# alexgittens/libskylark

Measured on AMD Instinct MI355X. Metric: sketch+apply GB/s and randSVD wall-clock on 1e6×1e3 dense, 1/2/4/8 MI355X, higher is better.
Workload: dtype bf16; 1 GPU; model=FJLT + randomized rank-20 SVD (q=2) of dense bf16 1000000x1000, global_batch=1000000, seq_len=1000

## Files before the change

### libskylark_amd/_native/src/rsvd_engine.cpp

```cpp
#include <hip/hip_runtime.h>

#include <cstdlib>
#include <cstring>
#include <new>

#include "sl_common.hpp"

SL_API int sl_rsvd_pass_grid(int64_t m);
SL_API int64_t sl_rsvd_pass_workspace(int64_t m, int64_t n, int k);
SL_API int sl_rsvd_pass(const void* A, int64_t m, int64_t n, int64_t lda, const void* Zt, int k, void* ws, float* Y,
                        int64_t ldy, int final_pass, int variant, void* stream);
SL_API int sl_rsvd_reduce_z(const void* ws, int64_t m, int64_t n, int k, void* Wout, int w_f64, int ldw,
                            double* Gout, int ldg, int* zero_word, void* stream);
SL_API int sl_rsvd_make_v(const double* W, int n, int k, int ldw, const double* N, int r, float* V, const double* s64,
                          float* s32, void* stream);
SL_API int sl_rsvd_make_v_ind(const double* W, int n, int k, int ldw, const double* N, int r, const double* s64,
                              float* const* optr, void* stream);
SL_API int sl_rsvd_set_ptrs(float** tab, float* a, float* b, float* c, void* stream);
SL_API int64_t sl_rsvd_bnd_workspace(int k);
SL_API int sl_rsvd_bnd_coresident(int n, int k, int* ok);
SL_API int sl_rsvd_bnd_set_fault(const void* bws, int missing, uint64_t bound_ticks);
SL_API int sl_rsvd_boundary(int final_, int n, int k, int r, double* WG, void* bws, int* status, int status_or,
                            double* Rinv, void* Zt, float* M, double* N, double* s64, int* mirror, float* V,
                            float* s32, float* const* optr, void* stream);
SL_API int sl_tsk_f32_xm_ind(const float* Y, int64_t m, int k, const float* M, int k2, float* const* optr,
                             void* stream);
SL_API int sl_rsvd_fjlt_zt_tab(uint64_t seed, uint64_t baseD, uint64_t baseS, double scale, int k, int n, void* Zt,
                               float** tab, float* a, float* b, float* c, void* stream);
SL_API int sl_rsvd_fjlt_zt(uint64_t seed, uint64_t baseD, uint64_t baseS, double scale, int k, int n, void* Zt,
                           void* stream);
SL_API int sl_tsk_f32_xm(const float* Y, int64_t m, int k, int64_t ldy, const float* M, int k2, float* out,
                         int64_t ldo, double* G, void* ws, void* stream);
SL_API int sl_rsvd_zt_from_f64(const double* src, int64_t count, void* Zt, void* stream);
SL_API int sl_fill_random(void* out, int dtype, int dist, uint64_t seed, uint64_t base, int64_t rows, int64_t cols,
                          int64_t sr, int64_t sc, int64_t r0, int64_t c0, int64_t ir, int64_t ic, double p0, double p1,
                          double scale, int precise, void* stream);
SL_API int sl_comm_all_reduce(void* comm, const void* send, void* recv, int64_t count, int dtype, int op,
                              void* stream);

namespace {

struct Plan {
  int64_t m = 0, n = 0, lda = 0;
  int k = 0, r = 0, q = 0;
  char* base = nullptr;
  void* pass_ws = nullptr;
  uint16_t* Zt = nullptr;
  double* WG = nullptr;
  float* Y = nullptr;
  void* bnd_ws = nullptr;
  float* last_ptrs[3] = {nullptr, nullptr, nullptr};
  hipStream_t last_ptrs_stream = nullptr;
  bool fjlt_pending = false;
  uint64_t fj_seed = 0, fj_baseD = 0, fj_baseS = 0;
  double fj_scale = 0.0;
  double* Rinv = nullptr;
  float* M = nullptr;
  double* N = nullptr;
  double* s64 = nullptr;
  float** optr = nullptr;
  int* status = nullptr;
  int* mirror_host = nullptr;
  int* mirror_dev = nullptr;
  hipGraph_t graph[2] = {nullptr, nullptr};
  hipGraphExec_t exec[2] = {nullptr, nullptr};
  const void* graph_A = nullptr;
  hipStream_t cap_stream = nullptr;
  hipEvent_t cap_ev = nullptr;
};

int64_t align256(int64_t b) { return (b + 255) & ~(int64_t)255; }

int pass_nt_code() {
  static int c = -1;
  if (c < 0) {
    const char* e = std::getenv("SL_PASS_NT");
    c = e ? (std::atoi(e) & 7) : 0;
  }
  return c;
}

int pass_nt_final_code() {
  static int c = -1;
  if (c < 0) {
    const char* e = std::getenv("SL_PASS_NT_FINAL");
    c = e ? (std::atoi(e) & 7) : -1;
    if (c < 0) c = 8;
  }
  return c == 8 ? pass_nt_code() : c;
}

int flush_fjlt(Plan* p, hipStream_t s, float** tab = nullptr, float* a = nullptr, float* b = nullptr,
               float* c = nullptr) {
  if (!p->fjlt_pending) return SL_OK;
  p->fjlt_pending = false;
  return sl_rsvd_fjlt_zt_tab(p->fj_seed, p->fj_baseD, p->fj_baseS, p->fj_scale, p->k, (int)p->n, p->Zt, tab, a, b,
                             c, s);
}

int seg(Plan* p, const void* A, int i, hipStream_t s, float* V = nullptr, float* s32 = nullptr,
        float* const* optr = nullptr) {
  const bool final_pass = i == p->q;
  if (i > p->q + 1 || i < 0) { sl_set_last_error("rsvd: segment out of range"); return SL_ERR_INVALID; }
  int rc = SL_OK;
  if (i > 0) {
    const int fin = i == p->q + 1 ? 1 : 0;
    rc = sl_rsvd_boundary(fin, (int)p->n, p->k, p->r, p->WG, p->bnd_ws, p->status, 1, p->Rinv, p->Zt, p->M, p->N,
                          p->s64, p->mirror_dev, V, s32, optr, s);
    if (rc != SL_OK || fin) return rc;
  }
  rc = sl_rsvd_pass(A, p->m, p->n, p->lda, p->Zt, p->k, p->pass_ws, final_pass ? p->Y : nullptr, p->k,
                    final_pass ? 1 : 0, ((i & 1) ? 256 : 0) | ((final_pass ? pass_nt_final_code() : pass_nt_code()) << 9),
                    s);
  if (rc != SL_OK) return rc;
  return sl_rsvd_reduce_z(p->pass_ws, p->m, p->n, p->k, p->WG, 1, p->k, final_pass ? p->WG + p->n * p->k : nullptr,
                          p->k, i == 0 ? p->status : nullptr, s);
}

void drop_graph(Plan* p) {
  for (int v = 0; v < 2; ++v) {
    if (p->exec[v]) (void)hipGraphExecDestroy(p->exec[v]);
    if (p->graph[v]) (void)hipGraphDestroy(p->graph[v]);
    p->exec[v] = nullptr;
    p->graph[v] = nullptr;
  }
  p->graph_A = nullptr;
}

int finish_ind(Plan* p, hipStream_t s) {
  return sl_tsk_f32_xm_ind(p->Y, p->m, p->k, p->M, p->r, p->optr, s);
}

int capture(Plan* p, const void* A, int with_finish, hipStream_t st) {
  if (!p->cap_stream) {
    SL_HIP_CHECK(hipStreamCreateWithFlags(&p->cap_stream, hipStreamNonBlocking));
    SL_HIP_CHECK(hipEventCreateWithFlags(&p->cap_ev, hipEventDisableTiming));
  }
  SL_HIP_CHECK(hipEventRecord(p->cap_ev, st));
  SL_HIP_CHECK(hipStreamWaitEvent(p->cap_stream, p->cap_ev, 0));
  SL_HIP_CHECK(hipStreamSynchronize(p->cap_stream));
  hipStream_t cst = p->cap_stream;
  SL_HIP_CHECK(hipStreamBeginCapture(cst, hipStreamCaptureModeThreadLocal));
  int rc = SL_OK;
  for (int i = 0; i <= p->q + 1 && rc == SL_OK; ++i)
    rc = seg(p, A, i, cst, nullptr, nullptr, with_finish ? p->optr : nullptr);
  if (rc == SL_OK && with_finish) rc = finish_ind(p, cst);
  hipGraph_t g = nullptr;
  const hipError_t e = hipStreamEndCapture(cst, &g);
  if (rc != SL_OK || e != hipSuccess) {
    if (g) (void)hipGraphDestroy(g);
    if (rc == SL_OK) { sl_set_last_error(hipGetErrorString(e)); rc = SL_ERR_HIP; }
    return rc;
  }
  hipGraphExec_t ex = nullptr;
  if (hipGraphInstantiate(&ex, g, nullptr, nullptr, 0) != hipSuccess) {
    (void)hipGraphDestroy(g);
    sl_set_last_error("rsvd_run: graph instantiate failed");
    return SL_ERR_HIP;
  }
  p->graph[with_finish] = g;
  p->exec[with_finish] = ex;
  p->graph_A = A;
  return SL_OK;
}

}

SL_API int sl_rsvd_plan_create(int64_t m, int64_t n, int64_t lda, int k, int r, int q, void** out) {
  *out = nullptr;
  if (m < 1 || n < 16 || n > 1024 || n % 8 || lda % 8 || k < 1 || k > 48 || r < 1 || r > k || q < 0) {
    sl_set_last_error("rsvd_plan: needs m >= 1, 16 <= n <= 1024, n % 8 == 0, lda % 8 == 0, 1 <= r <= k <= 48, q >= 0");
    return SL_ERR_UNSUPPORTED;
  }
  {
    int ok = 0;
    const int rc = sl_rsvd_bnd_coresident((int)n, k, &ok);
    if (rc != SL_OK) return rc;
    if (!ok) return SL_ERR_UNSUPPORTED;
  }
  Plan* p = new (std::nothrow) Plan();
  if (!p) return SL_ERR_GENERIC;
  p->m = m; p->n = n; p->lda = lda; p->k = k; p->r = r; p->q = q;
  int64_t off = 0;
  const int64_t o_pass = off; off = align256(off + sl_rsvd_pass_workspace(m, n, k));
  const int64_t o_zt = off;   off = align256(off + n * k * 2);
  const int64_t o_wg = off;   off = align256(off + (n + k) * k * 8);
  const int64_t o_y = off;    off = align256(off + m * k * 4);
  const int64_t o_bnd = off;  off = align256(off + sl_rsvd_bnd_workspace(k));
  const int64_t o_ri = off;   off = align256(off + (int64_t)k * k * 8);
  const int64_t o_m = off;    off = align256(off + (int64_t)k * r * 4);
  const int64_t o_n = off;    off = align256(off + (int64_t)k * r * 8);
  const int64_t o_s = off;    off = align256(off + (int64_t)r * 8);
  const int64_t o_st = off;   off = align256(off + 16);
  const int64_t o_op = off;   off = align256(off + 4 * (int64_t)sizeof(float*));
  if (hipMalloc((void**)&p->base, (size_t)off) != hipSuccess) {
    delete p;
    sl_set_last_error("rsvd_plan: device allocation failed");
    return SL_ERR_HIP;
  }
  p->pass_ws = p->base + o_pass;
  p->Zt = (uint16_t*)(p->base + o_zt);
  p->WG = (double*)(p->base + o_wg);
  p->Y = (float*)(p->base + o_y);
  p->bnd_ws = p->base + o_bnd;
  p->Rinv = (double*)(p->base + o_ri);
  p->M = (float*)(p->base + o_m);
  p->N = (double*)(p->base + o_n);
  p->s64 = (double*)(p->base + o_s);
  p->status = (int*)(p->base + o_st);
  p->optr = (float**)(p->base + o_op);
  if (hipMemset(p->bnd_ws, 0, (size_t)sl_rsvd_bnd_workspace(k)) != hipSuccess ||
      hipMemset(p->status, 0, 16) != hipSuccess) {
    (void)hipFree(p->base);
    delete p;
    sl_set_last_error("rsvd_plan: memset failed");
    return SL_ERR_HIP;
  }
  if (hipHostMalloc((void**)&p->mirror_host, 64, hipHostMallocMapped) == hipSuccess) {
    *p->mirror_host = 0;
    if (hipHostGetDevicePointer((void**)&p->mirror_dev, p->mirror_host, 0) != hipSuccess) {
      (void)hipHostFree(p->mirror_host);
      p->mirror_host = p->mirror_dev = nullptr;
    }
  }
  *out = p;
  return SL_OK;
}

SL_API int sl_rsvd_plan_destroy(void* plan) {
  Plan* p = (Plan*)plan;
  if (!p) return SL_OK;
  drop_graph(p);
  (void)sl_rsvd_bnd_set_fault(p->bnd_ws, 0, 0);
  if (p->cap_ev) (void)hipEventDestroy(p->cap_ev);
  if (p->cap_stream) (void)hipStreamDestroy(p->cap_stream);
  if (p->mirror_host) (void)hipHostFree(p->mirror_host);
  (void)hipFree(p->base);
  delete p;
  return SL_OK;
}

SL_API int sl_rsvd_plan_bind(void* plan, double* WG, int* status) {
  Plan* p = (Plan*)plan;
  drop_graph(p);
  if (WG) p->WG = WG;
  if (status) p->status = status;
  return SL_OK;
}

SL_API int sl_rsvd_plan_set_fault(void* plan, int missing, uint64_t bound_ticks) {
  Plan* p = (Plan*)plan;
  drop_graph(p);
  return sl_rsvd_bnd_set_fault(p->bnd_ws, missing, bound_ticks);
}

SL_API int sl_rsvd_set_fjlt(void* plan, uint64_t seed, uint64_t baseD, uint64_t baseS, double scale, void* stream) {
  (void)stream;
  Plan* p = (Plan*)plan;
  p->fjlt_pending = true;
  p->fj_seed = seed; p->fj_baseD = baseD; p->fj_baseS = baseS; p->fj_scale = scale;
  return SL_OK;
}

SL_API int sl_rsvd_set_dense(void* plan, int dist, uint64_t seed, uint64_t base, double p0, double p1, double scale,
                             void* stream) {
  Plan* p = (Plan*)plan;
// ... 107 lines not shown
```

### libskylark_amd/_native/src/rsvd_pass.hip

```cpp
#include <algorithm>

#include "sl_common.hpp"

namespace {

typedef __attribute__((ext_vector_type(8))) __bf16 bf16x8;
typedef __attribute__((ext_vector_type(4))) short s16x4;
typedef __attribute__((ext_vector_type(8))) short s16x8;
typedef __attribute__((ext_vector_type(4))) float f32x4;
typedef __attribute__((ext_vector_type(4))) double f64x4;
typedef __attribute__((address_space(3))) void lds_void;
typedef __attribute__((address_space(3))) s16x4 lds_s16x4;


__device__ __forceinline__ void glds16(const void* gsrc, unsigned lds_base) {
  unsigned keep;
  asm volatile(
      "s_mov_b32 %0, m0\n\t"
      "s_mov_b32 m0, %2\n\t"
      "s_nop 0\n\t"
      "global_load_lds_dwordx4 %1, off\n\t"
      "s_mov_b32 m0, %0"
      : "=&s"(keep)
      : "v"(gsrc), "s"(lds_base)
      : "memory");
}

template <bool NT = false>
__device__ __forceinline__ void glds16s(unsigned voff, const void* sbase, unsigned lds_base) {
  unsigned keep;
  if constexpr (NT)
    asm volatile(
        "s_mov_b32 %0, m0\n\t"
        "s_mov_b32 m0, %3\n\t"
        "s_nop 0\n\t"
        "global_load_lds_dwordx4 %1, %2 nt\n\t"
        "s_mov_b32 m0, %0"
        : "=&s"(keep)
        : "v"(voff), "s"(sbase), "s"(lds_base)
        : "memory");
  else
    asm volatile(
        "s_mov_b32 %0, m0\n\t"
        "s_mov_b32 m0, %3\n\t"
        "s_nop 0\n\t"
        "global_load_lds_dwordx4 %1, %2\n\t"
        "s_mov_b32 m0, %0"
        : "=&s"(keep)
        : "v"(voff), "s"(sbase), "s"(lds_base)
        : "memory");
}

__device__ __forceinline__ void wait_vm(int n) {
  switch (n) {
#define SLW(N) case N: asm volatile("s_waitcnt vmcnt(" #N ")" ::: "memory"); break;
    SLW(0) SLW(1) SLW(2) SLW(3) SLW(4) SLW(5) SLW(6) SLW(7) SLW(8) SLW(9) SLW(10) SLW(11) SLW(12) SLW(13)
    SLW(14) SLW(15) SLW(16) SLW(17) SLW(18) SLW(19) SLW(20) SLW(21) SLW(22) SLW(23) SLW(24) SLW(25)
    SLW(26) SLW(27) SLW(28) SLW(29) SLW(30) SLW(31)
#undef SLW
    default: asm volatile("s_waitcnt vmcnt(0)" ::: "memory"); break;
  }
}

__device__ __forceinline__ void lds_barrier() {
  asm volatile("s_waitcnt lgkmcnt(0)" ::: "memory");
  __builtin_amdgcn_s_barrier();
  asm volatile("" ::: "memory");
}

template <int NCH>
__device__ __forceinline__ int swz4(int row) {
  if constexpr (NCH == 16) return ((row << 1) & 15) ^ (((row >> 3) & 1) * 9);
  else return row & (NCH - 1);
}


template <typename IT, typename OT>
__device__ __forceinline__ void reduce_body(const IT* __restrict__ slab, int nslab, int64_t total, int cols,
                                            OT* __restrict__ out, int ldo, int blk, double (*part)[128]) {
  const int lane = threadIdx.x & 63, v = threadIdx.x >> 6;
  const int64_t e0 = (int64_t)blk * 128 + 2 * lane;
  double a0 = 0, a1 = 0, b0 = 0, b1 = 0;
  if (e0 + 1 < total) {
    int s = v;
    for (; s + 56 < nslab; s += 64) {
      IT x0[8], x1[8];
#pragma unroll
      for (int q = 0; q < 8; ++q) {
        const IT* p = slab + (int64_t)(s + 8 * q) * total + e0;
        x0[q] = p[0];
        x1[q] = p[1];
      }
#pragma unroll
      for (int q = 0; q < 8; q += 2) {
        a0 += (double)x0[q]; a1 += (double)x1[q];
        b0 += (double)x0[q + 1]; b1 += (double)x1[q + 1];
      }
    }
    for (; s + 8 < nslab; s += 16) {
      const IT* p = slab + (int64_t)s * total + e0;
      const IT* q = p + 8 * total;
      a0 += (double)p[0]; a1 += (double)p[1];
      b0 += (double)q[0]; b1 += (double)q[1];
    }
    for (; s < nslab; s += 8) {
      const IT* p = slab + (int64_t)s * total + e0;
      a0 += (double)p[0]; a1 += (double)p[1];
    }
  } else if (e0 < total) {
    for (int s = v; s < nslab; s += 8) a0 += (double)slab[(int64_t)s * total + e0];
  }
  part[v][2 * lane] = a0 + b0;
  part[v][2 * lane + 1] = a1 + b1;
  __syncthreads();
  if (threadIdx.x < 128) {
    const int64_t e = (int64_t)blk * 128 + threadIdx.x;
    if (e < total) {
      double sum = 0;
#pragma unroll
      for (int u = 0; u < 8; ++u) sum += part[u][threadIdx.x];
      const int64_t i = e / cols, j = e - i * cols;
      out[i * ldo + j] = (OT)sum;
    }
  }
}

template <typename IT, typename OT>
__global__ void __launch_bounds__(512)
k_rsvd_reduce(const IT* __restrict__ slab, int nslab, int64_t total, int cols, OT* __restrict__ out, int ldo,
              int* __restrict__ zero_word) {
  __shared__ double part[8][128];
  if (zero_word && blockIdx.x == 0 && threadIdx.x == 0) *zero_word = 0;
  reduce_body<IT, OT>(slab, nslab, total, cols, out, ldo, blockIdx.x, part);
}

__global__ void __launch_bounds__(512)
k_rsvd_reduce_wg(const float* __restrict__ wslab, int64_t tw, int cols, double* __restrict__ wout, int ldw,
                 const double* __restrict__ gslab, int64_t tg, double* __restrict__ gout, int ldg, int nslab, int gw,
                 int* __restrict__ zero_word) {
  __shared__ double part[8][128];
  if (zero_word && blockIdx.x == 0 && threadIdx.x == 0) *zero_word = 0;
  if ((int)blockIdx.x < gw) reduce_body<float, double>(wslab, nslab, tw, cols, wout, ldw, blockIdx.x, part);
  else reduce_body<double, double>(gslab, nslab, tg, cols, gout, ldg, blockIdx.x - gw, part);
}

struct P5Tiles {
  int base[8];
  int cnt[8];
  int gown[8];
  int prio;
  int rev;
  int nt;
  int ntail;
  int nty;
  int kx;
  const float* D;
  int64_t lddc;
};

#ifndef P1_PD
#define P1_PD 8
#endif
#ifndef P3_PT
#define P3_PT 4
#endif
constexpr int P5_NBUF = 4, P5_BM = 16, P5_ROWB = 256, P5_REGION = 4096, P5_LPB = 4, P5_T1 = 2, P5_T2 = 12,
              P5_GS = 2;

template <int KT>
constexpr int p5_y16p() { return 16 * KT * P5_BM * 2 + 16; }
template <int KT, bool FINAL, int EXT = 0>
constexpr int p5_lds() {
  return P5_NBUF * 8 * P5_REGION + 4 * p5_y16p<KT>() + (FINAL ? 2 * P5_BM * 16 * KT * 4 : 0) +
         (EXT == 2 ? P5_NBUF * P5_BM * 16 * 4 : 0);
}

template <int KT, bool FINAL, bool GRAM, bool YROLE, int TM, int KS, int EXT>
__device__ __forceinline__ void p5_body(const bf16_t* __restrict__ A, int64_t m, int n, int64_t lda,
                                        const bf16_t* __restrict__ Zt, int k, float* __restrict__ Wslab,
                                        double* __restrict__ Gslab, float* __restrict__ Y, int64_t ldy,
                                        float* __restrict__ scratch, const P5Tiles& pt, char* smem, const int w) {
  constexpr int KP = 16 * KT, BM = P5_BM, NBUF = P5_NBUF, ROWB = P5_ROWB, REGION = P5_REGION, LPB = P5_LPB;
  constexpr int Y16P = p5_y16p<KT>();
  char* ring = smem;
  char* y16b = smem + NBUF * 8 * REGION;
  float* yfb = (float*)(y16b + 4 * Y16P);
  float* dsl = yfb + 2 * BM * KP;
  const int kr = EXT ? pt.kx : k;
  const int lane = threadIdx.x & 63;
  const int g4 = lane >> 4, i16 = lane & 15;
  const int64_t nblocks = (m + BM - 1) / BM;
  const int64_t b0 = blockIdx.x, bstep = gridDim.x;
  const int64_t nloc = b0 < nblocks ? (nblocks - 1 - b0) / bstep + 1 : 0;
  const bool rev = pt.rev != 0;
  auto row0 = [&](int64_t jb) -> int64_t {
    const int64_t b = b0 + jb * bstep;
    return (rev ? nblocks - 1 - b : b) * BM;
  };
  const bool dma_on = 128 * w < n;
  const int tbase = pt.base[w], tcnt = pt.cnt[w];
  if (!dma_on) {
    for (int sl = 0; sl < NBUF; ++sl)
      for (int o = lane * 16; o < REGION; o += 1024) *(f32x4*)(ring + (sl * 8 + w) * REGION + o) = f32x4{0.f, 0.f, 0.f, 0.f};
  }

  bf16x8 zf[YROLE ? KS : 1];
  if constexpr (YROLE) {
#pragma unroll
    for (int ks = 0; ks < KS; ++ks) {
      const int col = 16 * w + i16, kk = 32 * ks + 8 * g4;
      bf16x8 v = {};
      if (col < k && kk + 8 <= n) v = *(const bf16x8*)(Zt + (int64_t)col * n + kk);
      zf[ks] = v;
    }
#pragma unroll
    for (int ks = 0; ks < KS; ++ks) asm volatile("" ::"v"(zf[ks]));
  }
  asm volatile("s_waitcnt vmcnt(0)" ::: "memory");

  f32x4 accW[TM > 0 ? TM : 1][KT];
#pragma unroll
  for (int a = 0; a < TM; ++a)
#pragma unroll
    for (int t = 0; t < KT; ++t) accW[a][t] = f32x4{0.f, 0.f, 0.f, 0.f};
  constexpr bool G_ON = GRAM && !YROLE;
  f64x4 accG[G_ON ? P5_GS : 1];
  f32x4 gblk[G_ON ? P5_GS : 1];
#pragma unroll
  for (int s = 0; s < (G_ON ? P5_GS : 1); ++s) {
    accG[s] = f64x4{0.0, 0.0, 0.0, 0.0};
    gblk[s] = f32x4{0.f, 0.f, 0.f, 0.f};
  }
  constexpr int GT = KT * (KT + 1) / 2;
  const int gfirst = pt.gown[w] & 0xff, gstride = pt.gown[w] >> 8;
  bool gpend = false;
  auto gram_acc = [&]() {
    if constexpr (G_ON) {
      if (gpend) {
#pragma unroll
        for (int s = 0; s < P5_GS; ++s)
#pragma unroll
          for (int e = 0; e < 4; ++e) accG[s][e] += (double)gblk[s][e];
      }
    }
  };

  unsigned voff[LPB];
#pragma unroll
  for (int i = 0; i < LPB; ++i) {
    const int byte = i * 1024 + lane * 16;
    const int row = byte / ROWB;
    const int sl = (byte % ROWB) / 16;
    const int chunk = sl ^ swz4<16>(row);
    int col = 128 * w + chunk * 8;
    col = col + 8 <= n ? col : n - 8;
    voff[i] = (unsigned)((row * lda + col) * 2);
  }
  auto issue = [&](int64_t blk) {
    if (!dma_on) return;
    const int slot = (int)(blk % NBUF);
    char* region = ring + (slot * 8 + w) * REGION;
    const int64_t r0 = row0(blk);
    if (r0 + BM <= m) {
      const bf16_t* base = A + r0 * lda;
      if (pt.nt && blk < nloc - pt.ntail) {
#pragma unroll
        for (int i = 0; i < LPB; ++i) {
          const unsigned dst = __builtin_amdgcn_readfirstlane((unsigned)(uintptr_t)(lds_void*)(region + i * 1024));
          glds16s<true>(voff[i], (const void*)base, dst);
        }
      } else {
#pragma unroll
        for (int i = 0; i < LPB; ++i) {
          const unsigned dst = __builtin_amdgcn_readfirstlane((unsigned)(uintptr_t)(lds_void*)(region + i * 1024));
          glds16s<false>(voff[i], (const void*)base, dst);
        }
      }
      if constexpr (EXT == 2) {
        if (w == 0) {
          const int c = lane >> 2, rq = lane & 3;
          const float* src = pt.D + (c < kr ? (int64_t)c * pt.lddc + r0 + 4 * rq : 0);
          const unsigned dst = __builtin_amdgcn_readfirstlane((unsigned)(uintptr_t)(lds_void*)(dsl + slot * BM * 16));
          glds16((const void*)src, dst);
        }
      }
    } else {
#pragma unroll
      for (int i = 0; i < LPB; ++i) {
        const int byte = i * 1024 + lane * 16;
        const int row = byte / ROWB;
        int64_t grow = r0 + row;
        grow = grow < m ? grow : m - 1;
        const unsigned dst = __builtin_amdgcn_readfirstlane((unsigned)(uintptr_t)(lds_void*)(region + i * 1024));
        glds16((const void*)((const char*)(A + grow * lda) + (voff[i] - (unsigned)(row * lda * 2))), dst);
      }
    }
  };
  const int lpb = dma_on ? (EXT == 2 && w == 0 ? LPB + 1 : LPB) : 0;

  auto step1 = [&](int64_t jb) {
    if constexpr (YROLE) {
      const char* reg0 = ring + (int)(jb % NBUF) * 8 * REGION;
      const int sw = swz4<16>(i16);
      auto rd = [&](int ks) -> bf16x8 {
        const int chunk = ((ks & 3) << 2) + g4;
        return *(const bf16x8*)(reg0 + (ks >> 2) * REGION + i16 * ROWB + ((chunk ^ sw) << 4));
      };
      f32x4 acc = {0.f, 0.f, 0.f, 0.f};
      if constexpr (FINAL) {
#pragma unroll
        for (int ks = 0; ks < KS; ++ks) acc = __builtin_amdgcn_mfma_f32_16x16x32_bf16(rd(ks), zf[ks], acc, 0, 0, 0);
      } else {
        constexpr int PD = P1_PD < KS ? P1_PD : KS;
        __builtin_amdgcn_sched_barrier(0);
        bf16x8 afr[PD];
#pragma unroll
        for (int u = 0; u < PD; ++u) afr[u] = rd(u);
        f32x4 acc0 = {0.f, 0.f, 0.f, 0.f}, acc1 = {0.f, 0.f, 0.f, 0.f};
#pragma unroll
        for (int ks = 0; ks < KS; ++ks) {
          const bf16x8 af = afr[ks % PD];
          if (ks & 1) acc1 = __builtin_amdgcn_mfma_f32_16x16x32_bf16(af, zf[ks], acc1, 0, 0, 0);
          else acc0 = __builtin_amdgcn_mfma_f32_16x16x32_bf16(af, zf[ks], acc0, 0, 0, 0);
          if (ks + PD < KS) afr[ks % PD] = rd(ks + PD);
        }
        __builtin_amdgcn_sched_group_barrier(0x100, PD, 0);
#pragma unroll
        for (int ks = 0; ks + PD < KS; ++ks) {
          __builtin_amdgcn_sched_group_barrier(0x008, 1, 0);
          __builtin_amdgcn_sched_group_barrier(0x100, 1, 0);
        }
        __builtin_amdgcn_sched_group_barrier(0x008, PD, 0);
        __builtin_amdgcn_sched_barrier(0);
        acc = acc0 + acc1;
      }
      const int64_t r0 = row0(jb);
      if (r0 + BM > m) {
#pragma unroll
        for (int e = 0; e < 4; ++e)
          if (r0 + 4 * g4 + e >= m) acc[e] = 0.f;
      }
      f32x4 yfold = acc;
      if constexpr (EXT != 0) {
#pragma unroll
        for (int e = 0; e < 4; ++e) {
          const float part = __shfl_down(acc[e], kr, 16);
          yfold[e] = i16 < kr ? acc[e] + part : 0.f;
        }
        acc = yfold;
        if constexpr (EXT == 2) {
          const float* dsp = dsl + (int)(jb % NBUF) * BM * 16;
#pragma unroll
          for (int e = 0; e < 4; ++e) acc[e] = i16 < kr ? dsp[i16 * 16 + 4 * g4 + e] : 0.f;
        }
      }
      unsigned hb[4], lb[4];
      float yv[4];
#pragma unroll
      for (int e = 0; e < 4; ++e) {
        hb[e] = f_to_bf16(acc[e]);
        const float hv = __uint_as_float(hb[e] << 16);
        lb[e] = f_to_bf16(acc[e] - hv);
        yv[e] = hv + __uint_as_float(lb[e] << 16);
      }
      char* y16 = y16b + (int)(jb & 1) * 2 * Y16P;
      const int col = 16 * w + i16;
      *(uint2*)(y16 + col * 32 + g4 * 8) = make_uint2(hb[0] | (hb[1] << 16), hb[2] | (hb[3] << 16));
      *(uint2*)(y16 + Y16P + col * 32 + g4 * 8) = make_uint2(lb[0] | (lb[1] << 16), lb[2] | (lb[3] << 16));
      s16x4 hi, lo;
#pragma unroll
      for (int e = 0; e < 4; ++e) {
        hi[e] = (short)hb[e];
        lo[e] = (short)lb[e];
      }
      if constexpr (FINAL) {
        float* yf = yfb + (int)(jb & 1) * BM * KP;
        if (col < kr) {
#pragma unroll
          for (int e = 0; e < 4; ++e) yf[(4 * g4 + e) * kr + col] = EXT ? yfold[e] : yv[e];
        }
      }
    }
  };

  const bool vecY = FINAL && (kr % 4 == 0) && (ldy == kr);
  const int wy = YROLE ? -1 : w - KT;
  const int nyv = (BM * kr + (vecY ? 255 : 63)) / (vecY ? 256 : 64);
  const int nst = (!FINAL || wy < 0 || wy >= nyv) ? 0 : (nyv - wy + (8 - KT) - 1) / (8 - KT);
  auto store_y = [&](int64_t jb) {
    if constexpr (FINAL && !YROLE) {
      const float* yf = yfb + (int)(jb & 1) * BM * KP;
      const int64_t r0 = row0(jb);
      for (int q = wy; q < nyv; q += 8 - KT) {
        if (vecY) {
          const int t = q * 64 + lane;
          const bool ok = t < BM * kr / 4 && r0 + (4 * t) / kr < m;
          f32x4 v = {0.f, 0.f, 0.f, 0.f};
          if (ok) v = *(const f32x4*)&yf[4 * t];
          float* dst = ok ? Y + r0 * ldy + 4 * t : scratch + 4 * lane;
          if (pt.nty) __builtin_nontemporal_store(v, (f32x4*)dst);
          else *(f32x4*)dst = v;
        } else {
          const int t = q * 64 + lane;
          const int row = t / kr, col = t - (t / kr) * kr;
          const bool ok = t < BM * kr && r0 + row < m;
          const float v = ok ? yf[t] : 0.f;
          float* dst = ok ? Y + (r0 + row) * ldy + col : scratch + lane;
          *dst = v;
        }
      }
    }
  };

  auto step3 = [&](int64_t j) {
    const char* slotp = ring + (int)(j % NBUF) * 8 * REGION;
    const char* y16 = y16b + (int)(j & 1) * 2 * Y16P;
    const int rb = 8 * (g4 >> 1);
    const char* yp = y16 + (g4 & 1) * Y16P + rb * 2;
    bf16x8 yfr[KT];
#pragma unroll
    for (int t = 0; t < KT; ++t) yfr[t] = *(const bf16x8*)(yp + (16 * t + i16) * 32);
    if constexpr (G_ON) {
#pragma unroll
      for (int sg = 0; sg < P5_GS; ++sg) {
        const int tau = gfirst + sg * gstride;
        if (gstride == 0 || tau >= GT) break;
        const int t1 = tau < KT ? 0 : (tau < 2 * KT - 1 ? 1 : 2);
        const int t2 = t1 == 0 ? tau : (t1 == 1 ? tau - KT + 1 : 2);
        bf16x8 y1 = yfr[0], y2 = yfr[0];
#pragma unroll
        for (int t = 1; t < KT; ++t) {
          y1 = t1 == t ? yfr[t] : y1;
          y2 = t2 == t ? yfr[t] : y2;
        }
        const bf16x8 ysw = *(const bf16x8*)(y16 + ((g4 & 1) ^ 1) * Y16P + rb * 2 + (16 * t2 + i16) * 32);
        const f32x4 z4 = {0.f, 0.f, 0.f, 0.f};
        gblk[sg] = __builtin_amdgcn_mfma_f32_16x16x32_bf16(y1, y2, z4, 0, 0, 0);
        gblk[sg] = __builtin_amdgcn_mfma_f32_16x16x32_bf16(y1, ysw, gblk[sg], 0, 0, 0);
      }
      gpend = true;
    }
    (void)GT;
    const int q = i16 >> 2, p = i16 & 3;
    auto tile_rd = [&](int ct) -> bf16x8 {
      const int gt = tbase + (YROLE || ct < tcnt ? ct : 0);
      const char* region = slotp + (gt >> 3) * REGION;
      const int chunk = 2 * (gt & 7) + (p >> 1);
      const int ra = rb + q, rbb = rb + 4 + q;
      const char* aa = region + ra * ROWB + ((chunk ^ swz4<16>(ra)) << 4) + (p & 1) * 8;
      const char* ab2 = region + rbb * ROWB + ((chunk ^ swz4<16>(rbb)) << 4) + (p & 1) * 8;
      const s16x4 a4 = __builtin_amdgcn_ds_read_tr16_b64_v4i16((lds_s16x4*)aa);
      const s16x4 b4 = __builtin_amdgcn_ds_read_tr16_b64_v4i16((lds_s16x4*)ab2);
      s16x8 a8;
#pragma unroll
      for (int u = 0; u < 4; ++u) {
        a8[u] = a4[u];
        a8[4 + u] = b4[u];
      }
      return __builtin_bit_cast(bf16x8, a8);
    };
    if constexpr (FINAL) {
#pragma unroll
      for (int ct = 0; ct < TM; ++ct) {
        const bf16x8 af8 = tile_rd(ct);
#pragma unroll
        for (int t = 0; t < KT; ++t) accW[ct][t] = __builtin_amdgcn_mfma_f32_16x16x32_bf16(af8, yfr[t], accW[ct][t], 0, 0, 0);
      }
    } else if constexpr (TM > 0) {
      constexpr int PT = P3_PT < TM ? P3_PT : TM;
      __builtin_amdgcn_sched_barrier(0);
      bf16x8 tfr[PT];
#pragma unroll
      for (int u = 0; u < PT; ++u) tfr[u] = tile_rd(u);
#pragma unroll
      for (int ct = 0; ct < TM; ++ct) {
        const bf16x8 af8 = tfr[ct % PT];
#pragma unroll
        for (int t = 0; t < KT; ++t) accW[ct][t] = __builtin_amdgcn_mfma_f32_16x16x32_bf16(af8, yfr[t], accW[ct][t], 0, 0, 0);
        if (ct + PT < TM) tfr[ct % PT] = tile_rd(ct + PT);
      }
      __builtin_amdgcn_sched_group_barrier(0x100, 2 * PT, 1);
#pragma unroll
      for (int ct = 0; ct + PT < TM; ++ct) {
        __builtin_amdgcn_sched_group_barrier(0x008, KT, 1);
        __builtin_amdgcn_sched_group_barrier(0x100, 2, 1);
      }
      __builtin_amdgcn_sched_group_barrier(0x008, KT * PT, 1);
      __builtin_amdgcn_sched_barrier(0);
    }
  };

#pragma unroll
  for (int b = 0; b < NBUF - 1; ++b)
    if (b < nloc) issue(b);
  if (nloc > 0) wait_vm(lpb * ((1 < nloc) + (2 < nloc)));
  lds_barrier();
  if (nloc > 0) step1(0);

  for (int64_t j = 0; j < nloc; ++j) {
    if (j + 1 < nloc) wait_vm(lpb * (j + 2 < nloc) + nst * (int)(j < 2 ? j : 2));
    lds_barrier();
    gram_acc();
    if (j + NBUF - 1 < nloc) issue(j + NBUF - 1);
    if constexpr (FINAL && !YROLE) store_y(j);
    if (j + 1 < nloc) step1(j + 1);
    step3(j);
  }
  gram_acc();
  asm volatile("s_waitcnt vmcnt(0)" ::: "memory");

  {
    float* ws = Wslab + (int64_t)blockIdx.x * n * kr;
#pragma unroll
    for (int ct = 0; ct < TM; ++ct)
      if (ct < tcnt) {
        const int gt = tbase + ct;
#pragma unroll
        for (int t = 0; t < KT; ++t)
#pragma unroll
          for (int e = 0; e < 4; ++e) {
            const int row = 16 * gt + 4 * g4 + e, col = 16 * t + i16;
            if (row < n && col < kr) ws[(int64_t)row * kr + col] = accW[ct][t][e];
          }
      }
  }
  if constexpr (G_ON) {
    double* gs = Gslab + (int64_t)blockIdx.x * k * k;
#pragma unroll
    for (int sg = 0; sg < P5_GS; ++sg) {
      const int tau = gfirst + sg * gstride;
      if (gstride == 0 || tau >= GT) break;
      const int t1 = tau < KT ? 0 : (tau < 2 * KT - 1 ? 1 : 2);
      const int t2 = t1 == 0 ? tau : (t1 == 1 ? tau - KT + 1 : 2);
#pragma unroll
      for (int r = 0; r < 4; ++r) {
        const int i = 16 * t1 + 4 * g4 + r, jj = 16 * t2 + i16;
        if (i < k && jj < k && (t1 != t2 || i <= jj)) {
          gs[i * k + jj] = accG[sg][r];
          if (i != jj) gs[jj * k + i] = accG[sg][r];
        }
      }
    }
  }
}

template <int KT, bool FINAL, bool GRAM, int KS, int EXT = 0>
__global__ void __launch_bounds__(512, 1)
k_rsvd_pass5(const bf16_t* __restrict__ A, int64_t m, int n, int64_t lda, const bf16_t* __restrict__ Zt, int k,
             float* __restrict__ Wslab, double* __restrict__ Gslab, float* __restrict__ Y, int64_t ldy,
             float* __restrict__ scratch, P5Tiles pt) {
  extern __shared__ __attribute__((aligned(16))) char smem[];
  const int w = __builtin_amdgcn_readfirstlane(threadIdx.x >> 6);
  if (w < KT) {
    if (pt.prio == 1) __builtin_amdgcn_s_setprio(1);
    else if (pt.prio >= 2) __builtin_amdgcn_s_setprio(2);
    const int yt = pt.cnt[0];
    if (yt == 0)
      p5_body<KT, FINAL, GRAM, true, 0, KS, EXT>(A, m, n, lda, Zt, k, Wslab, Gslab, Y, ldy, scratch, pt, smem, w);
    else if (yt == 1)
      p5_body<KT, FINAL, GRAM, true, 1, KS, EXT>(A, m, n, lda, Zt, k, Wslab, Gslab, Y, ldy, scratch, pt, smem, w);
    else
      p5_body<KT, FINAL, GRAM, true, 2, KS, EXT>(A, m, n, lda, Zt, k, Wslab, Gslab, Y, ldy, scratch, pt, smem, w);
  } else {
    p5_body<KT, FINAL, GRAM, false, P5_T2, KS, EXT>(A, m, n, lda, Zt, k, Wslab, Gslab, Y, ldy, scratch, pt, smem, w);
  }
}

bool p5_tiles(int n, int KT, P5Tiles* pt) {
  const int nt16 = (n + 15) / 16, nks = (n + 31) / 32, nw = 8 - KT;
  int best = 1 << 30, bestT1 = -1;
  for (int T1 = 0; T1 <= P5_T1; ++T1) {
    const int rem = nt16 - KT * T1;
    if (rem < 0) break;
    const int T2 = (rem + nw - 1) / nw;
    if (T2 > P5_T2) continue;
    int cnt[8];
    int left = rem;
    for (int w = 0; w < 8; ++w) {
      if (w < KT) { cnt[w] = T1; continue; }
      cnt[w] = left < T2 ? left : T2;
      left -= cnt[w];
    }
    int worst = 0;
    for (int w = 0; w < 4; ++w) {
      auto load = [&](int v) { return (v < KT ? nks : 0) + KT * cnt[v]; };
      worst = std::max(worst, load(w) + load(w + 4));
    }
    if (worst < best) { best = worst; bestT1 = T1; }
  }
  if (bestT1 < 0) return false;
  const int rem = nt16 - KT * bestT1, T2 = (rem + nw - 1) / nw;
  int left = rem, base = 0;
  for (int w = 0; w < 8; ++w) {
    const int c = w < KT ? bestT1 : (left < T2 ? left : T2);
    if (w >= KT) left -= c;
    pt->base[w] = base;
    pt->cnt[w] = c;
    base += c;
  }
  const int GT = KT * (KT + 1) / 2;
  for (int w = 0; w < 8; ++w) {
    const int wi = w - KT;
    const bool own = wi >= 0 && wi < GT;
    pt->gown[w] = own ? (wi | (nw << 8)) : 0;
    if (own && (GT - wi + nw - 1) / nw > P5_GS) return false;
  }
  return true;
}

template <int KT, bool FINAL, bool GRAM>
int launch_pass5(const bf16_t* A, int64_t m, int n, int64_t lda, const bf16_t* Zt, int k, float* Wslab, double* Gslab,
                 float* Y, int64_t ldy, float* scratch, int grid, hipStream_t s, int variant) {
  P5Tiles pt{};
  pt.prio = (variant >> 6) & 3;
  pt.rev = (variant >> 8) & 1;
  {
    const int c = (variant >> 9) & 7;
    pt.nt = c != 0;
    pt.ntail = c >= 2 ? 8 * (c - 1) : 0;
  }
  pt.nty = (variant >> 12) & 1;
  if (!p5_tiles(n, KT, &pt)) {
    sl_set_last_error("rsvd_pass: no tile split for this n / k");
    return SL_ERR_UNSUPPORTED;
  }
  constexpr int LDS = p5_lds<KT, FINAL>();
  static_assert(LDS <= 160 * 1024, "LDS budget");
  if (n > 512) {
    SL_LDS_ATTR((k_rsvd_pass5<KT, FINAL, GRAM, 32>), LDS);
    k_rsvd_pass5<KT, FINAL, GRAM, 32><<<grid, 512, LDS, s>>>(A, m, n, lda, Zt, k, Wslab, Gslab, Y, ldy, scratch, pt);
  } else {
    SL_LDS_ATTR((k_rsvd_pass5<KT, FINAL, GRAM, 16>), LDS);
    k_rsvd_pass5<KT, FINAL, GRAM, 16><<<grid, 512, LDS, s>>>(A, m, n, lda, Zt, k, Wslab, Gslab, Y, ldy, scratch, pt);
  }
  SL_LAUNCH_CHECK();
  return SL_OK;
}

template <int EXT>
int launch_pass5_ext(const bf16_t* A, int64_t m, int n, int64_t lda, const bf16_t* Zt2, int kx, float* Wslab,
                     float* Y, int64_t ldy, const float* D, int64_t lddc, float* scratch, int grid, hipStream_t s,
                     int variant) {
  P5Tiles pt{};
  pt.prio = (variant >> 6) & 3;
  pt.rev = (variant >> 8) & 1;
  pt.kx = kx;
  pt.D = D;
  pt.lddc = lddc;
  if (!p5_tiles(n, 1, &pt)) {
    sl_set_last_error("rsvd_pass_ext: no tile split for this n");
    return SL_ERR_UNSUPPORTED;
  }
  constexpr int LDS = p5_lds<1, true, EXT>();
  static_assert(LDS <= 160 * 1024, "LDS budget");
  if (n > 512) {
    SL_LDS_ATTR((k_rsvd_pass5<1, true, false, 32, EXT>), LDS);
    k_rsvd_pass5<1, true, false, 32, EXT><<<grid, 512, LDS, s>>>(A, m, n, lda, Zt2, 2 * kx, Wslab, nullptr, Y, ldy,
                                                                 scratch, pt);
  } else {
    SL_LDS_ATTR((k_rsvd_pass5<1, true, false, 16, EXT>), LDS);
    k_rsvd_pass5<1, true, false, 16, EXT><<<grid, 512, LDS, s>>>(A, m, n, lda, Zt2, 2 * kx, Wslab, nullptr, Y, ldy,
                                                                 scratch, pt);
  }
  SL_LAUNCH_CHECK();
  return SL_OK;
}

int cu_count() {
  static int ncu = -1;
  if (ncu < 0) {
    int dev = 0;
    if (hipGetDevice(&dev) != hipSuccess ||
        hipDeviceGetAttribute(&ncu, hipDeviceAttributeMultiprocessorCount, dev) != hipSuccess)
      ncu = 256;
  }
  return ncu;
}

}

SL_API int sl_rsvd_pass_grid(int64_t m) {
  const int64_t nb = (m + 15) / 16;
  const int64_t c = cu_count();
  return (int)(nb < c ? (nb > 0 ? nb : 1) : c);
}

SL_API int64_t sl_rsvd_pass_workspace(int64_t m, int64_t n, int k) {
  const int64_t g = sl_rsvd_pass_grid(m);
  int64_t b = g * n * k * 4;
  b = (b + 255) & ~(int64_t)255;
  b += g * (int64_t)k * k * 8;
  b = (b + 255) & ~(int64_t)255;
  return b + 1024;
}

SL_API int sl_rsvd_pass(const void* A, int64_t m, int64_t n, int64_t lda, const void* Zt, int k, void* ws,
                        float* Y, int64_t ldy, int final_pass, int variant, void* stream) {
  if (m <= 0) return SL_OK;
  if (n % 8 || lda % 8 || n > 1024 || n < 16 || k < 1 || k > 48 || (final_pass && (!Y || ldy < k))) {
    sl_set_last_error("rsvd_pass: needs n % 8 == 0, lda % 8 == 0, 16 <= n <= 1024, 1 <= k <= 48 (and Y when final)");
    return SL_ERR_UNSUPPORTED;
  }
  hipStream_t s = (hipStream_t)stream;
  const int grid = sl_rsvd_pass_grid(m);
  char* base = (char*)ws;
  float* Wslab = (float*)base;
  int64_t off = ((int64_t)grid * n * k * 4 + 255) & ~(int64_t)255;
  double* Gslab = (double*)(base + off);
  off += (int64_t)grid * k * k * 8;
  off = (off + 255) & ~(int64_t)255;
  float* scratch = (float*)(base + off);
  const bf16_t* a = (const bf16_t*)A;
  const bf16_t* z = (const bf16_t*)Zt;
  const int KT = (k + 15) / 16;
#define SL_P5(KTT)                                                                                                 \
  return final_pass == 1 ? launch_pass5<KTT, true, true>(a, m, (int)n, lda, z, k, Wslab, Gslab, Y, ldy, scratch, grid, s, variant) \
       : final_pass == 2 ? launch_pass5<KTT, true, false>(a, m, (int)n, lda, z, k, Wslab, Gslab, Y, ldy, scratch, grid, s, variant) \
                         : launch_pass5<KTT, false, false>(a, m, (int)n, lda, z, k, Wslab, Gslab, Y, ldy, scratch, grid, s, variant)
  switch (KT) {
    case 1: SL_P5(1);
    case 2: SL_P5(2);
    default: SL_P5(3);
  }
#undef SL_P5
}

SL_API int sl_rsvd_pass_ext(const void* A, int64_t m, int64_t n, int64_t lda, const void* Zt2, int kx, void* ws,
                            float* Y, int64_t ldy, const float* D, int64_t lddc, int variant, void* stream) {
  if (m <= 0) return SL_OK;
  if (n % 8 || lda % 8 || n > 1024 || n < 16 || kx < 1 || kx > 8 || !Y || ldy < kx ||
      (D && (m % 16 || lddc % 4 || ((uintptr_t)D & 15) || lddc < m))) {
    sl_set_last_error("rsvd_pass_ext: needs n % 8 == 0, lda % 8 == 0, 16 <= n <= 1024, 1 <= kx <= 8, Y; "
                      "D: m % 16 == 0, lddc % 4 == 0, 16-B aligned");
    return SL_ERR_UNSUPPORTED;
  }
  const int grid = sl_rsvd_pass_grid(m);
  char* base = (char*)ws;
  int64_t off = ((int64_t)grid * n * kx * 4 + 255) & ~(int64_t)255;
  off += (int64_t)grid * kx * kx * 8;
  off = (off + 255) & ~(int64_t)255;
  float* scratch = (float*)(base + off);
  const bf16_t* a = (const bf16_t*)A;
  const bf16_t* z = (const bf16_t*)Zt2;
  hipStream_t s = (hipStream_t)stream;
  return D ? launch_pass5_ext<2>(a, m, (int)n, lda, z, kx, (float*)base, Y, ldy, D, lddc, scratch, grid, s, variant)
           : launch_pass5_ext<1>(a, m, (int)n, lda, z, kx, (float*)base, Y, ldy, nullptr, 0, scratch, grid, s, variant);
}

SL_API int sl_rsvd_reduce_z(const void* ws, int64_t m, int64_t n, int k, void* Wout, int w_f64, int ldw,
                            double* Gout, int ldg, int* zero_word, void* stream) {
  hipStream_t s = (hipStream_t)stream;
  const int grid = sl_rsvd_pass_grid(m);
  const char* base = (const char*)ws;
  const int64_t tw = n * k;
  const unsigned gw = (unsigned)((tw + 127) / 128);
  if (Gout && w_f64) {
    const int64_t off = ((int64_t)grid * n * k * 4 + 255) & ~(int64_t)255;
    const int64_t tg = (int64_t)k * k;
    const unsigned gg = (unsigned)((tg + 127) / 128);
    k_rsvd_reduce_wg<<<gw + gg, 512, 0, s>>>((const float*)base, tw, k, (double*)Wout, ldw,
                                              (const double*)(base + off), tg, Gout, ldg, grid, (int)gw, zero_word);
    SL_LAUNCH_CHECK();
    return SL_OK;
  }
  if (w_f64)
    k_rsvd_reduce<float, double><<<gw, 512, 0, s>>>((const float*)base, grid, tw, k, (double*)Wout, ldw, zero_word);
  else
    k_rsvd_reduce<float, float><<<gw, 512, 0, s>>>((const float*)base, grid, tw, k, (float*)Wout, ldw, zero_word);
  SL_LAUNCH_CHECK();
  if (Gout) {
    const int64_t off = ((int64_t)grid * n * k * 4 + 255) & ~(int64_t)255;
    const int64_t tg = (int64_t)k * k;
    k_rsvd_reduce<double, double><<<(unsigned)((tg + 127) / 128), 512, 0, s>>>((const double*)(base + off), grid, tg,
                                                                               k, Gout, ldg, nullptr);
    SL_LAUNCH_CHECK();
  }
  return SL_OK;
}

SL_API int sl_rsvd_reduce(const void* ws, int64_t m, int64_t n, int k, void* Wout, int w_f64, int ldw,
                          double* Gout, int ldg, void* stream) {
  return sl_rsvd_reduce_z(ws, m, n, k, Wout, w_f64, ldw, Gout, ldg, nullptr, stream);
}
```

Measured before the change: 1468 GB/s.

## Dedicate a service wave to Gram accumulation and Y stores in final pass

In the final (Gram) form of the fused rSVD pass, one wave (w=7) becomes a service wave that computes the full triangular Gram block set and does all Y stores, with a smaller tile count. The other waves keep only W tiles, and the final-pass MFMA chain uses a single accumulator. The tile splitter now searches T2 to balance the service wave's extra Gram cost against the W-tile waves. This replaces the earlier spread of Gram tiles across waves and drops the SL_PASS_NT_FINAL and nontemporal Y store options, trading a lighter load on most waves for a possible serial bottleneck on the service wave.

```diff
diff --git a/libskylark_amd/_native/src/rsvd_engine.cpp b/libskylark_amd/_native/src/rsvd_engine.cpp
--- a/libskylark_amd/_native/src/rsvd_engine.cpp
+++ b/libskylark_amd/_native/src/rsvd_engine.cpp
@@ -80,16 +80,6 @@
   return c;
 }
 
-int pass_nt_final_code() {
-  static int c = -1;
-  if (c < 0) {
-    const char* e = std::getenv("SL_PASS_NT_FINAL");
-    c = e ? (std::atoi(e) & 7) : -1;
-    if (c < 0) c = 8;
-  }
-  return c == 8 ? pass_nt_code() : c;
-}
-
 int flush_fjlt(Plan* p, hipStream_t s, float** tab = nullptr, float* a = nullptr, float* b = nullptr,
                float* c = nullptr) {
   if (!p->fjlt_pending) return SL_OK;
@@ -110,8 +100,7 @@
     if (rc != SL_OK || fin) return rc;
   }
   rc = sl_rsvd_pass(A, p->m, p->n, p->lda, p->Zt, p->k, p->pass_ws, final_pass ? p->Y : nullptr, p->k,
-                    final_pass ? 1 : 0, ((i & 1) ? 256 : 0) | ((final_pass ? pass_nt_final_code() : pass_nt_code()) << 9),
-                    s);
+                    final_pass ? 1 : 0, ((i & 1) ? 256 : 0) | (pass_nt_code() << 9), s);
   if (rc != SL_OK) return rc;
   return sl_rsvd_reduce_z(p->pass_ws, p->m, p->n, p->k, p->WG, 1, p->k, final_pass ? p->WG + p->n * p->k : nullptr,
                           p->k, i == 0 ? p->status : nullptr, s);
diff --git a/libskylark_amd/_native/src/rsvd_pass.hip b/libskylark_amd/_native/src/rsvd_pass.hip
--- a/libskylark_amd/_native/src/rsvd_pass.hip
+++ b/libskylark_amd/_native/src/rsvd_pass.hip
@@ -147,12 +147,10 @@
 struct P5Tiles {
   int base[8];
   int cnt[8];
-  int gown[8];
   int prio;
   int rev;
   int nt;
   int ntail;
-  int nty;
   int kx;
   const float* D;
   int64_t lddc;
@@ -164,8 +162,9 @@
 #ifndef P3_PT
 #define P3_PT 4
 #endif
-constexpr int P5_NBUF = 4, P5_BM = 16, P5_ROWB = 256, P5_REGION = 4096, P5_LPB = 4, P5_T1 = 2, P5_T2 = 12,
-              P5_GS = 2;
+constexpr int P5_NBUF = 4, P5_BM = 16, P5_ROWB = 256, P5_REGION = 4096, P5_LPB = 4, P5_T1 = 2, P5_T2 = 12;
+constexpr int P5_SVCW = 7, P5_T2F = 13, P5_TS = 6;
+enum { P5_ROLE_W = 0, P5_ROLE_Y = 1, P5_ROLE_SVC = 2 };
 
 template <int KT>
 constexpr int p5_y16p() { return 16 * KT * P5_BM * 2 + 16; }
@@ -175,13 +174,17 @@
          (EXT == 2 ? P5_NBUF * P5_BM * 16 * 4 : 0);
 }
 
-template <int KT, bool FINAL, bool GRAM, bool YROLE, int TM, int KS, int EXT>
+template <int KT, bool FINAL, bool GRAM, int ROLE, int TM, int KS, int EXT>
 __device__ __forceinline__ void p5_body(const bf16_t* __restrict__ A, int64_t m, int n, int64_t lda,
                                         const bf16_t* __restrict__ Zt, int k, float* __restrict__ Wslab,
                                         double* __restrict__ Gslab, float* __restrict__ Y, int64_t ldy,
                                         float* __restrict__ scratch, const P5Tiles& pt, char* smem, const int w) {
   constexpr int KP = 16 * KT, BM = P5_BM, NBUF = P5_NBUF, ROWB = P5_ROWB, REGION = P5_REGION, LPB = P5_LPB;
   constexpr int Y16P = p5_y16p<KT>();
+  constexpr bool YROLE = ROLE == P5_ROLE_Y, SVC = ROLE == P5_ROLE_SVC;
+  constexpr bool SVCF = GRAM;
+  static_assert(!GRAM || (FINAL && EXT == 0), "the Gram belongs to the final = 1 form");
+  static_assert(!SVC || SVCF, "service wave only in the service form");
   char* ring = smem;
   char* y16b = smem + NBUF * 8 * REGION;
   float* yfb = (float*)(y16b + 4 * Y16P);
@@ -223,25 +226,21 @@
   for (int a = 0; a < TM; ++a)
 #pragma unroll
     for (int t = 0; t < KT; ++t) accW[a][t] = f32x4{0.f, 0.f, 0.f, 0.f};
-  constexpr bool G_ON = GRAM && !YROLE;
-  f64x4 accG[G_ON ? P5_GS : 1];
-  f32x4 gblk[G_ON ? P5_GS : 1];
-#pragma unroll
-  for (int s = 0; s < (G_ON ? P5_GS : 1); ++s) {
+  constexpr bool G_ON = GRAM && SVC;
+  constexpr int GT = KT * (KT + 1) / 2;
+  f64x4 accG[G_ON ? GT : 1];
+  f32x4 gblk[G_ON ? GT : 1];
+#pragma unroll
+  for (int s = 0; s < (G_ON ? GT : 1); ++s) {
     accG[s] = f64x4{0.0, 0.0, 0.0, 0.0};
     gblk[s] = f32x4{0.f, 0.f, 0.f, 0.f};
   }
-  constexpr int GT = KT * (KT + 1) / 2;
-  const int gfirst = pt.gown[w] & 0xff, gstride = pt.gown[w] >> 8;
-  bool gpend = false;
   auto gram_acc = [&]() {
     if constexpr (G_ON) {
-      if (gpend) {
-#pragma unroll
-        for (int s = 0; s < P5_GS; ++s)
-#pragma unroll
-          for (int e = 0; e < 4; ++e) accG[s][e] += (double)gblk[s][e];
-      }
+#pragma unroll
+      for (int s = 0; s < GT; ++s)
+#pragma unroll
+        for (int e = 0; e < 4; ++e) accG[s][e] += (double)gblk[s][e];
     }
   };
 
@@ -307,7 +306,7 @@
         return *(const bf16x8*)(reg0 + (ks >> 2) * REGION + i16 * ROWB + ((chunk ^ sw) << 4));
       };
       f32x4 acc = {0.f, 0.f, 0.f, 0.f};
-      if constexpr (FINAL) {
+      if constexpr (FINAL && !SVCF) {
 #pragma unroll
         for (int ks = 0; ks < KS; ++ks) acc = __builtin_amdgcn_mfma_f32_16x16x32_bf16(rd(ks), zf[ks], acc, 0, 0, 0);
       } else {
@@ -320,7 +319,7 @@
 #pragma unroll
         for (int ks = 0; ks < KS; ++ks) {
           const bf16x8 af = afr[ks % PD];
-          if (ks & 1) acc1 = __builtin_amdgcn_mfma_f32_16x16x32_bf16(af, zf[ks], acc1, 0, 0, 0);
+          if (!FINAL && (ks & 1)) acc1 = __builtin_amdgcn_mfma_f32_16x16x32_bf16(af, zf[ks], acc1, 0, 0, 0);
           else acc0 = __builtin_amdgcn_mfma_f32_16x16x32_bf16(af, zf[ks], acc0, 0, 0, 0);
           if (ks + PD < KS) afr[ks % PD] = rd(ks + PD);
         }
@@ -332,7 +331,8 @@
         }
         __builtin_amdgcn_sched_group_barrier(0x008, PD, 0);
         __builtin_amdgcn_sched_barrier(0);
-        acc = acc0 + acc1;
+        if constexpr (FINAL) acc = acc0;
+        else acc = acc0 + acc1;
       }
       const int64_t r0 = row0(jb);
       if (r0 + BM > m) {
@@ -383,24 +383,42 @@
     }
   };
 
+  constexpr bool STORES = FINAL && (SVCF ? SVC : !YROLE);
   const bool vecY = FINAL && (kr % 4 == 0) && (ldy == kr);
-  const int wy = YROLE ? -1 : w - KT;
+  const int nsw = SVCF ? 1 : 8 - KT;
+  const int wy = !STORES ? -1 : (SVCF ? 0 : w - KT);
   const int nyv = (BM * kr + (vecY ? 255 : 63)) / (vecY ? 256 : 64);
-  const int nst = (!FINAL || wy < 0 || wy >= nyv) ? 0 : (nyv - wy + (8 - KT) - 1) / (8 - KT);
+  const int nst = (wy < 0 || wy >= nyv) ? 0 : (nyv - wy + nsw - 1) / nsw;
   auto store_y = [&](int64_t jb) {
-    if constexpr (FINAL && !YROLE) {
+    if constexpr (STORES) {
       const float* yf = yfb + (int)(jb & 1) * BM * KP;
       const int64_t r0 = row0(jb);
-      for (int q = wy; q < nyv; q += 8 - KT) {
-        if (vecY) {
+      if (vecY && SVCF) {
+        f32x4 v[3];
+        bool ok[3];
+#pragma unroll
+        for (int u = 0; u < 3; ++u) {
+          const int t = u * 64 + lane;
+          ok[u] = t < BM * kr / 4 && r0 + (4 * t) / kr < m;
+          v[u] = f32x4{0.f, 0.f, 0.f, 0.f};
+          if (ok[u]) v[u] = *(const f32x4*)&yf[4 * t];
+        }
+#pragma unroll
+        for (int u = 0; u < 3; ++u) {
+          const int t = u * 64 + lane;
+          if (u < nyv) *(f32x4*)(ok[u] ? Y + r0 * ldy + 4 * t : scratch + 4 * lane) = v[u];
+        }
+      } else if (vecY) {
+        for (int q = wy; q < nyv; q += nsw) {
           const int t = q * 64 + lane;
           const bool ok = t < BM * kr / 4 && r0 + (4 * t) / kr < m;
           f32x4 v = {0.f, 0.f, 0.f, 0.f};
           if (ok) v = *(const f32x4*)&yf[4 * t];
           float* dst = ok ? Y + r0 * ldy + 4 * t : scratch + 4 * lane;
-          if (pt.nty) __builtin_nontemporal_store(v, (f32x4*)dst);
-          else *(f32x4*)dst = v;
-        } else {
+          *(f32x4*)dst = v;
+        }
+      } else {
+        for (int q = wy; q < nyv; q += nsw) {
           const int t = q * 64 + lane;
           const int row = t / kr, col = t - (t / kr) * kr;
           const bool ok = t < BM * kr && r0 + row < m;
@@ -421,26 +439,21 @@
 #pragma unroll
     for (int t = 0; t < KT; ++t) yfr[t] = *(const bf16x8*)(yp + (16 * t + i16) * 32);
     if constexpr (G_ON) {
-#pragma unroll
-      for (int sg = 0; sg < P5_GS; ++sg) {
-        const int tau = gfirst + sg * gstride;
-        if (gstride == 0 || tau >= GT) break;
-        const int t1 = tau < KT ? 0 : (tau < 2 * KT - 1 ? 1 : 2);
-        const int t2 = t1 == 0 ? tau : (t1 == 1 ? tau - KT + 1 : 2);
-        bf16x8 y1 = yfr[0], y2 = yfr[0];
-#pragma unroll
-        for (int t = 1; t < KT; ++t) {
-          y1 = t1 == t ? yfr[t] : y1;
-          y2 = t2 == t ? yfr[t] : y2;
-        }
-        const bf16x8 ysw = *(const bf16x8*)(y16 + ((g4 & 1) ^ 1) * Y16P + rb * 2 + (16 * t2 + i16) * 32);
-        const f32x4 z4 = {0.f, 0.f, 0.f, 0.f};
-        gblk[sg] = __builtin_amdgcn_mfma_f32_16x16x32_bf16(y1, y2, z4, 0, 0, 0);
-        gblk[sg] = __builtin_amdgcn_mfma_f32_16x16x32_bf16(y1, ysw, gblk[sg], 0, 0, 0);
-      }
-      gpend = true;
-    }
-    (void)GT;
+      bf16x8 ysw[KT];
+#pragma unroll
+      for (int t = 0; t < KT; ++t)
+        ysw[t] = *(const bf16x8*)(y16 + ((g4 & 1) ^ 1) * Y16P + rb * 2 + (16 * t + i16) * 32);
+#pragma unroll
+      for (int sweep = 0; sweep < 2; ++sweep)
+#pragma unroll
+        for (int tau = 0; tau < GT; ++tau) {
+          const int t1 = tau < KT ? 0 : (tau < 2 * KT - 1 ? 1 : 2);
+          const int t2 = t1 == 0 ? tau : (t1 == 1 ? tau - KT + 1 : 2);
+          const f32x4 z4 = {0.f, 0.f, 0.f, 0.f};
+          gblk[tau] = sweep == 0 ? __builtin_amdgcn_mfma_f32_16x16x32_bf16(yfr[t1], yfr[t2], z4, 0, 0, 0)
+                                 : __builtin_amdgcn_mfma_f32_16x16x32_bf16(yfr[t1], ysw[t2], gblk[tau], 0, 0, 0);
+        }
+    }
     const int q = i16 >> 2, p = i16 & 3;
     auto tile_rd = [&](int ct) -> bf16x8 {
       const int gt = tbase + (YROLE || ct < tcnt ? ct : 0);
@@ -459,7 +472,7 @@
       }
       return __builtin_bit_cast(bf16x8, a8);
     };
-    if constexpr (FINAL) {
+    if constexpr (FINAL && !SVCF) {
 #pragma unroll
       for (int ct = 0; ct < TM; ++ct) {
         const bf16x8 af8 = tile_rd(ct);
@@ -502,7 +515,7 @@
     lds_barrier();
     gram_acc();
     if (j + NBUF - 1 < nloc) issue(j + NBUF - 1);
-    if constexpr (FINAL && !YROLE) store_y(j);
+    store_y(j);
     if (j + 1 < nloc) step1(j + 1);
     step3(j);
   }
@@ -527,17 +540,15 @@
   if constexpr (G_ON) {
     double* gs = Gslab + (int64_t)blockIdx.x * k * k;
 #pragma unroll
-    for (int sg = 0; sg < P5_GS; ++sg) {
-      const int tau = gfirst + sg * gstride;
-      if (gstride == 0 || tau >= GT) break;
+    for (int tau = 0; tau < GT; ++tau) {
       const int t1 = tau < KT ? 0 : (tau < 2 * KT - 1 ? 1 : 2);
       const int t2 = t1 == 0 ? tau : (t1 == 1 ? tau - KT + 1 : 2);
 #pragma unroll
       for (int r = 0; r < 4; ++r) {
         const int i = 16 * t1 + 4 * g4 + r, jj = 16 * t2 + i16;
         if (i < k && jj < k && (t1 != t2 || i <= jj)) {
-          gs[i * k + jj] = accG[sg][r];
-          if (i != jj) gs[jj * k + i] = accG[sg][r];
+          gs[i * k + jj] = accG[tau][r];
+          if (i != jj) gs[jj * k + i] = accG[tau][r];
         }
       }
     }
@@ -556,54 +567,57 @@
     else if (pt.prio >= 2) __builtin_amdgcn_s_setprio(2);
     const int yt = pt.cnt[0];
     if (yt == 0)
-      p5_body<KT, FINAL, GRAM, true, 0, KS, EXT>(A, m, n, lda, Zt, k, Wslab, Gslab, Y, ldy, scratch, pt, smem, w);
+      p5_body<KT, FINAL, GRAM, P5_ROLE_Y, 0, KS, EXT>(A, m, n, lda, Zt, k, Wslab, Gslab, Y, ldy, scratch, pt, smem, w);
     else if (yt == 1)
-      p5_body<KT, FINAL, GRAM, true, 1, KS, EXT>(A, m, n, lda, Zt, k, Wslab, Gslab, Y, ldy, scratch, pt, smem, w);
+      p5_body<KT, FINAL, GRAM, P5_ROLE_Y, 1, KS, EXT>(A, m, n, lda, Zt, k, Wslab, Gslab, Y, ldy, scratch, pt, smem, w);
     else
-      p5_body<KT, FINAL, GRAM, true, 2, KS, EXT>(A, m, n, lda, Zt, k, Wslab, Gslab, Y, ldy, scratch, pt, smem, w);
+      p5_body<KT, FINAL, GRAM, P5_ROLE_Y, 2, KS, EXT>(A, m, n, lda, Zt, k, Wslab, Gslab, Y, ldy, scratch, pt, smem, w);
+  } else if constexpr (GRAM) {
+    if (w == P5_SVCW)
+      p5_body<KT, FINAL, GRAM, P5_ROLE_SVC, P5_TS, KS, EXT>(A, m, n, lda, Zt, k, Wslab, Gslab, Y, ldy, scratch, pt, smem, w);
+    else
+      p5_body<KT, FINAL, GRAM, P5_ROLE_W, P5_T2F, KS, EXT>(A, m, n, lda, Zt, k, Wslab, Gslab, Y, ldy, scratch, pt, smem, w);
   } else {
-    p5_body<KT, FINAL, GRAM, false, P5_T2, KS, EXT>(A, m, n, lda, Zt, k, Wslab, Gslab, Y, ldy, scratch, pt, smem, w);
-  }
-}
-
-bool p5_tiles(int n, int KT, P5Tiles* pt) {
-  const int nt16 = (n + 15) / 16, nks = (n + 31) / 32, nw = 8 - KT;
-  int best = 1 << 30, bestT1 = -1;
+    p5_body<KT, FINAL, GRAM, P5_ROLE_W, P5_T2, KS, EXT>(A, m, n, lda, Zt, k, Wslab, Gslab, Y, ldy, scratch, pt, smem, w);
+  }
+}
+
+bool p5_tiles(int n, int KT, bool svc, P5Tiles* pt) {
+  const int nt16 = (n + 15) / 16, nks = (n + 31) / 32;
+  const int nh = (svc ? 7 : 8) - KT;
+  const int gcost = svc ? KT * (KT + 1) : 0;
+  auto split = [&](int T1, int T2, int* cnt) {
+    int left = nt16 - KT * T1;
+    for (int w = 0; w < 8; ++w) {
+      if (w < KT) { cnt[w] = T1; continue; }
+      cnt[w] = w < KT + nh ? std::min(left, T2) : left;
+      left -= cnt[w];
+    }
+    return left == 0 && cnt[7] <= (svc ? P5_TS : T2);
+  };
+  int best = 1 << 30, bestS = 1 << 30, bestT1 = -1, bestT2 = -1;
   for (int T1 = 0; T1 <= P5_T1; ++T1) {
     const int rem = nt16 - KT * T1;
     if (rem < 0) break;
-    const int T2 = (rem + nw - 1) / nw;
-    if (T2 > P5_T2) continue;
-    int cnt[8];
-    int left = rem;
-    for (int w = 0; w < 8; ++w) {
-      if (w < KT) { cnt[w] = T1; continue; }
-      cnt[w] = left < T2 ? left : T2;
-      left -= cnt[w];
-    }
-    int worst = 0;
-    for (int w = 0; w < 4; ++w) {
-      auto load = [&](int v) { return (v < KT ? nks : 0) + KT * cnt[v]; };
-      worst = std::max(worst, load(w) + load(w + 4));
-    }
-    if (worst < best) { best = worst; bestT1 = T1; }
+    for (int T2 = svc ? 0 : (rem + nh - 1) / nh; T2 <= (svc ? P5_T2F : P5_T2); ++T2) {
+      int cnt[8];
+      if (split(T1, T2, cnt)) {
+        int worst = 0;
+        for (int w = 0; w < 4; ++w) {
+          auto load = [&](int v) { return (v < KT ? nks : 0) + KT * cnt[v] + (svc && v == P5_SVCW ? gcost : 0); };
+          worst = std::max(worst, load(w) + load(w + 4));
+        }
+        const int S = svc ? cnt[P5_SVCW] : 0;
+        if (worst < best || (worst == best && S < bestS)) { best = worst; bestS = S; bestT1 = T1; bestT2 = T2; }
+      }
+      if (!svc) break;
+    }
   }
   if (bestT1 < 0) return false;
-  const int rem = nt16 - KT * bestT1, T2 = (rem + nw - 1) / nw;
-  int left = rem, base = 0;
-  for (int w = 0; w < 8; ++w) {
-    const int c = w < KT ? bestT1 : (left < T2 ? left : T2);
-    if (w >= KT) left -= c;
+  split(bestT1, bestT2, pt->cnt);
+  for (int w = 0, base = 0; w < 8; ++w) {
     pt->base[w] = base;
-    pt->cnt[w] = c;
-    base += c;
-  }
-  const int GT = KT * (KT + 1) / 2;
-  for (int w = 0; w < 8; ++w) {
-    const int wi = w - KT;
-    const bool own = wi >= 0 && wi < GT;
-    pt->gown[w] = own ? (wi | (nw << 8)) : 0;
-    if (own && (GT - wi + nw - 1) / nw > P5_GS) return false;
+    base += pt->cnt[w];
   }
   return true;
 }
@@ -619,8 +633,7 @@
     pt.nt = c != 0;
     pt.ntail = c >= 2 ? 8 * (c - 1) : 0;
   }
-  pt.nty = (variant >> 12) & 1;
-  if (!p5_tiles(n, KT, &pt)) {
+  if (!p5_tiles(n, KT, GRAM, &pt)) {
     sl_set_last_error("rsvd_pass: no tile split for this n / k");
     return SL_ERR_UNSUPPORTED;
   }
@@ -647,7 +660,7 @@
   pt.kx = kx;
   pt.D = D;
   pt.lddc = lddc;
-  if (!p5_tiles(n, 1, &pt)) {
+  if (!p5_tiles(n, 1, false, &pt)) {
     sl_set_last_error("rsvd_pass_ext: no tile split for this n");
     return SL_ERR_UNSUPPORTED;
   }
```

Measured after the change: 1467 GB/s. Within noise of the previous version (-0.1%).
